# Yotsuei/ClearConverse

Measured on AMD Instinct MI355X. Metric: xRT (audio-sec/wall-sec) end-to-end, 30 s 16 kHz clips, higher is better.
Workload: dtype bf16

## Files before the change

### clearconverse_amd/csrc/sepformer.hip

```cpp
#include <math.h>
#include "../../include/ccx.h"
#include "ccx_common.h"
#include "elementwise.h"
#include <type_traits>
#include "gemm_bf16.h"
#include "model_store.h"

namespace {

typedef __attribute__((ext_vector_type(4))) short bf16x4v;

__global__ __launch_bounds__(256) void sep_encoder_kernel(const float* __restrict__ mix, long mix_stride,
                                                          const int* __restrict__ tok_utt, const int* __restrict__ tok_pos,
                                                          const int* __restrict__ utt_L, const float* __restrict__ w,
                                                          float* __restrict__ feats, int n_tok) {
  const int tok = blockIdx.x * 4 + (threadIdx.x >> 6), lane = threadIdx.x & 63;
  if (tok >= n_tok) return;
  const int u = tok_utt[tok], l = tok_pos[tok];
  float2 o = make_float2(0.f, 0.f);
  if (l < utt_L[u]) {
    const float* x = mix + (long)u * mix_stride + 8 * l;
    float xs[16];
#pragma unroll
    for (int k = 0; k < 16; k++) xs[k] = x[k];
    float a = 0.f, b = 0.f;
#pragma unroll
    for (int k = 0; k < 16; k++) {
      a = fmaf(w[(2 * lane) * 16 + k], xs[k], a);
      b = fmaf(w[(2 * lane + 1) * 16 + k], xs[k], b);
    }
    o = make_float2(fmaxf(a, 0.f), fmaxf(b, 0.f));
  }
  ((float2*)(feats + (long)tok * 128))[lane] = o;
}

__global__ void sep_block_input_kernel(const float* __restrict__ x, const float* __restrict__ hc, const int* __restrict__ tok_seq,
                                       const int* __restrict__ tok_pos, const float* __restrict__ pe, float* __restrict__ xin,
                                       float* __restrict__ h, int n_tok) {
  const long i = (long)blockIdx.x * blockDim.x + threadIdx.x;
  if (i >= (long)n_tok * 32) return;
  const int tok = (int)(i >> 5), c4 = (int)(i & 31);
  float4 v = ((const float4*)x)[i];
  if (hc) {
    const float4 a = ((const float4*)(hc + (long)tok_seq[tok] * 128))[c4];
    v.x += a.x; v.y += a.y; v.z += a.z; v.w += a.w;
  }
  ((float4*)xin)[i] = v;
  const float4 p = ((const float4*)(pe + (long)tok_pos[tok] * 128))[c4];
  ((float4*)h)[i] = make_float4(v.x + p.x, v.y + p.y, v.z + p.z, v.w + p.w);
}

__global__ __launch_bounds__(256, 2) void sep_attention_kernel(const bf16_t* __restrict__ qkv, const int* __restrict__ seq_start,
                                                            const int* __restrict__ seq_len, bf16_t* __restrict__ out,
                                                            float scale_log2e) {
  const int lane = threadIdx.x & 63, wave = threadIdx.x >> 6;
  const int seq = blockIdx.x, head = blockIdx.y * 4 + wave;
  const int s0 = seq_start[seq], len = seq_len[seq];
  const int l15 = lane & 15, h4 = lane >> 4;
  const int n_qt = (len + 15) >> 4, n_kt = n_qt;
  const bf16_t* base = qkv + (long)s0 * 384 + head * 16;

  auto load_k = [&](int kt) -> bf16x4v {
    int krow = kt * 16 + l15;
    krow = krow < len ? krow : len - 1;
    return *(const bf16x4v*)(base + 128 + (long)krow * 384 + 4 * h4);
  };
  auto load_v = [&](int kt) -> bf16x4v {
    bf16x4v v;
#pragma unroll
    for (int j = 0; j < 4; j++) {
      int vr = kt * 16 + 4 * h4 + j;
      vr = vr < len ? vr : len - 1;
      v[j] = (short)base[256 + (long)vr * 384 + l15];
    }
    return v;
  };
  const bool resident = n_kt <= 10;
  bf16x4v k_all[10], v_all[10];
  if (resident) {
#pragma unroll
    for (int t = 0; t < 10; t++) {
      const int kt = t < n_kt ? t : n_kt - 1;
      k_all[t] = load_k(kt);
      v_all[t] = load_v(kt);
    }
  }

  for (int qt = 0; qt < n_qt; qt++) {
    int qrow = qt * 16 + l15;
    qrow = qrow < len ? qrow : len - 1;
    const bf16x4v qf = *(const bf16x4v*)(base + (long)qrow * 384 + 4 * h4);
    float m_run = -1e30f, l_run = 0.f;
    f32x4 o = {0.f, 0.f, 0.f, 0.f};
    auto key_block = [&](int kt0, int nk, auto full_tag) {
      constexpr bool FULL = decltype(full_tag)::value;
      f32x4 s[10];
      bf16x4v vf[10];
#pragma unroll
      for (int t = 0; t < 10; t++) {
        if (FULL || t < nk) {
          const bf16x4v kf = resident ? k_all[t] : load_k(kt0 + t);
          s[t] = __builtin_amdgcn_mfma_f32_16x16x16bf16_1k(kf, qf, (f32x4){0.f, 0.f, 0.f, 0.f}, 0, 0, 0);
          vf[t] = resident ? v_all[t] : load_v(kt0 + t);
        }
      }
      float mx = -1e30f;
#pragma unroll
      for (int t = 0; t < 10; t++)
        if (FULL || t < nk) {
          if ((kt0 + t) * 16 + 16 > len) {
#pragma unroll
            for (int r = 0; r < 4; r++)
              if ((kt0 + t) * 16 + 4 * h4 + r >= len) s[t][r] = -INFINITY;
          }
#pragma unroll
          for (int r = 0; r < 4; r++) mx = fmaxf(mx, s[t][r]);
        }
      mx = fmaxf(mx, lane_xor16(mx));
      mx = fmaxf(mx, lane_xor32(mx));
      mx = fmaxf(m_run, mx * scale_log2e);
      const float alpha = __builtin_amdgcn_exp2f(m_run - mx);
      m_run = mx;
      float ps = 0.f;
#pragma unroll
      for (int t = 0; t < 10; t++)
        if (FULL || t < nk) {
#pragma unroll
          for (int r = 0; r < 4; r++) {
            const float pv = __builtin_amdgcn_exp2f(fmaf(s[t][r], scale_log2e, -mx));
            s[t][r] = pv;
            ps += pv;
          }
        }
      l_run = l_run * alpha + ps;
      float arow[4];
#pragma unroll
      for (int r = 0; r < 4; r++) arow[r] = __shfl(alpha, 4 * h4 + r, 64);
#pragma unroll
      for (int r = 0; r < 4; r++) o[r] *= arow[r];
#pragma unroll
      for (int t = 0; t < 10; t++)
        if (FULL || t < nk) {
          union { bf16x4v v; uint32_t u[2]; } pa;
          pa.u[0] = pack_bf16x2(s[t][0], s[t][1]);
          pa.u[1] = pack_bf16x2(s[t][2], s[t][3]);
          o = __builtin_amdgcn_mfma_f32_16x16x16bf16_1k(pa.v, vf[t], o, 0, 0, 0);
        }
    };
    for (int kt0 = 0; kt0 < n_kt; kt0 += 10) {
      const int nk = (n_kt - kt0) < 10 ? (n_kt - kt0) : 10;
      if (nk == 10) key_block(kt0, 10, std::true_type{});
      else key_block(kt0, nk, std::false_type{});
    }
    float lt = l_run + lane_xor16(l_run);
    lt += lane_xor32(lt);
#pragma unroll
    for (int r = 0; r < 4; r++) {
      const int q = qt * 16 + 4 * h4 + r;
      const float inv = 1.0f / __shfl(lt, 4 * h4 + r, 64);
      if (q < len) out[(long)(s0 + q) * 128 + head * 16 + l15] = f32_to_bf16(o[r] * inv);
    }
  }
}

__device__ __forceinline__ float2 ln_row128(const float* __restrict__ row, const float* __restrict__ g,
                                            const float* __restrict__ b, int lane) {
  const float2 v = ((const float2*)row)[lane];
  const float mean = wave_reduce_sum(v.x + v.y) * (1.0f / 128.0f);
  const float dx = v.x - mean, dy = v.y - mean;
  const float rstd = rsqrtf(wave_reduce_sum(dx * dx + dy * dy) * (1.0f / 128.0f) + 1e-6f);
  const float2 gg = ((const float2*)g)[lane], bb = ((const float2*)b)[lane];
  return make_float2(dx * rstd * gg.x + bb.x, dy * rstd * gg.y + bb.y);
}

__global__ __launch_bounds__(256) void sep_final_norm_kernel(const float* __restrict__ h, const float* __restrict__ xin,
                                                             const int* __restrict__ seq_start, const int* __restrict__ seq_len,
                                                             const float* __restrict__ ln_g, const float* __restrict__ ln_b,
                                                             const float* __restrict__ gln_g, const float* __restrict__ gln_b,
                                                             float* __restrict__ y) {
  __shared__ float red[8];
  const int seq = blockIdx.x, lane = threadIdx.x & 63, wave = threadIdx.x >> 6;
  const int s0 = seq_start[seq], len = seq_len[seq];
  float sum = 0.f;
  for (int r = wave; r < len; r += 4) {
    const float2 v = ln_row128(h + (long)(s0 + r) * 128, ln_g, ln_b, lane);
    sum += v.x + v.y;
  }
  sum = wave_reduce_sum(sum);
  if (lane == 0) red[wave] = sum;
  __syncthreads();
  const float n = (float)len * 128.0f;
  const float mean = (red[0] + red[1] + red[2] + red[3]) / n;
  float sq = 0.f;
  for (int r = wave; r < len; r += 4) {
    const float2 v = ln_row128(h + (long)(s0 + r) * 128, ln_g, ln_b, lane);
    sq += (v.x - mean) * (v.x - mean) + (v.y - mean) * (v.y - mean);
  }
  sq = wave_reduce_sum(sq);
  if (lane == 0) red[4 + wave] = sq;
  __syncthreads();
  const float rstd = 1.0f / sqrtf((red[4] + red[5] + red[6] + red[7]) / n + 1e-8f);
  const float2 gg = ((const float2*)gln_g)[lane], bb = ((const float2*)gln_b)[lane];
  for (int r = wave; r < len; r += 4) {
    const float2 v = ln_row128(h + (long)(s0 + r) * 128, ln_g, ln_b, lane);
    const float2 xi = ((const float2*)(xin + (long)(s0 + r) * 128))[lane];
    ((float2*)(y + (long)(s0 + r) * 128))[lane] =
        make_float2(gg.x * (v.x - mean) * rstd + bb.x + xi.x, gg.y * (v.y - mean) * rstd + bb.y + xi.y);
  }
}

#define FF_TOK 256
#define FF_HB 64
#define FF_P1 (FF_HB * 256)
#define FF_P2 (128 * FF_HB * 2)
#define FF_STAGE (FF_P1 + FF_P2)
#define FF_NSTAGE 4
#define FF_LDS (FF_NSTAGE * FF_STAGE + 4096)
typedef const __attribute__((address_space(1))) void* ff_gptr_t;
typedef __attribute__((address_space(3))) void* ff_lptr_t;

__device__ __forceinline__ int ff_key1(int r) { return (r & 3) | (((r >> 4) & 3) << 2); }
__device__ __forceinline__ int ff_key2(int r) { return ((r >> 1) & 1) | (((r >> 5) & 1) << 2); }

constexpr int AB_MAX_TOK = 160;
__device__ __forceinline__ int ab_off(int row, int chunk) { return row * 256 + ((chunk ^ (row & 15)) << 4); }

__global__ __launch_bounds__(512) void sep_attn_block_kernel(float* __restrict__ h, const float* __restrict__ ln_g, const float* __restrict__ ln_b,
                                                             const bf16_t* __restrict__ Wqkv, const float* __restrict__ bqkv,
                                                             const bf16_t* __restrict__ Wo, const float* __restrict__ bo,
                                                             const int* __restrict__ seq_start, const int* __restrict__ seq_len,
                                                             float scale_log2e, float eps) {
  __shared__ __attribute__((aligned(16))) char xs[AB_MAX_TOK * 256];
  const int tid = threadIdx.x, lane = tid & 63;
  const int wave = __builtin_amdgcn_readfirstlane(tid >> 6);
  const int l15 = lane & 15, h4 = lane >> 4;
  const int seq = blockIdx.x;
  const int s0 = seq_start[seq], len = seq_len[seq];
  if (len <= 0) return;
  const int n_t = (len + 15) >> 4;

  {
    const float2 g = ((const float2*)ln_g)[lane], b = ((const float2*)ln_b)[lane];
#pragma unroll
    for (int half = 0; half < 2; half++) {
      float2 v[10];
#pragma unroll
      for (int i = 0; i < 10; i++) {
        const int r = wave + 8 * (10 * half + i);
        v[i] = r < len ? ((const float2*)(h + (long)(s0 + r) * 128))[lane] : make_float2(0.f, 0.f);
      }
#pragma unroll
      for (int i = 0; i < 10; i++) {
        const int r = wave + 8 * (10 * half + i);
        const float mean = wave_reduce_sum(v[i].x + v[i].y) * (1.f / 128.f);
        const float dx = v[i].x - mean, dy = v[i].y - mean;
        const float rstd = rsqrtf(wave_reduce_sum(dx * dx + dy * dy) * (1.f / 128.f) + eps);
        uint32_t o = pack_bf16x2(dx * rstd * g.x + b.x, dy * rstd * g.y + b.y);
        if (r >= len) o = 0;
        *(uint32_t*)(xs + ab_off(r, lane >> 2) + (lane & 3) * 4) = o;
      }
    }
  }
  __syncthreads();

  bf16x4v q_all[10], k_all[10], v_all[10];
  {
    bf16x8 wq[4], wk[4];
#pragma unroll
    for (int ks = 0; ks < 4; ks++) {
      const long o = (long)(16 * wave + l15) * 128 + 32 * ks + 8 * h4;
      wq[ks] = *(const bf16x8*)(Wqkv + o);
      wk[ks] = *(const bf16x8*)(Wqkv + 128 * 128 + o);
    }
    const float4 bq = *(const float4*)(bqkv + 16 * wave + 4 * h4);
    const float4 bk = *(const float4*)(bqkv + 128 + 16 * wave + 4 * h4);
#pragma unroll
    for (int t = 0; t < 10; t++) {
      const int tt = t < n_t ? t : n_t - 1;
      f32x4 aq = {0.f, 0.f, 0.f, 0.f}, ak = aq;
#pragma unroll
      for (int ks = 0; ks < 4; ks++) {
        const bf16x8 xf = *(const bf16x8*)(xs + ab_off(16 * tt + l15, 4 * ks + h4));
        aq = __builtin_amdgcn_mfma_f32_16x16x32_bf16(wq[ks], xf, aq, 0, 0, 0);
        ak = __builtin_amdgcn_mfma_f32_16x16x32_bf16(wk[ks], xf, ak, 0, 0, 0);
      }
      union { bf16x4v v; uint32_t u[2]; } c;
      c.u[0] = pack_bf16x2(aq[0] + bq.x, aq[1] + bq.y); c.u[1] = pack_bf16x2(aq[2] + bq.z, aq[3] + bq.w);
      q_all[t] = c.v;
      c.u[0] = pack_bf16x2(ak[0] + bk.x, ak[1] + bk.y); c.u[1] = pack_bf16x2(ak[2] + bk.z, ak[3] + bk.w);
      k_all[t] = c.v;
    }
  }
  {
    bf16x8 wv[4];
#pragma unroll
    for (int ks = 0; ks < 4; ks++) wv[ks] = *(const bf16x8*)(Wqkv + 256 * 128 + (long)(16 * wave + l15) * 128 + 32 * ks + 8 * h4);
    const float bv = bqkv[256 + 16 * wave + l15];
#pragma unroll
    for (int t = 0; t < 10; t++) {
      const int tt = t < n_t ? t : n_t - 1;
      f32x4 av = {0.f, 0.f, 0.f, 0.f};
#pragma unroll
      for (int ks = 0; ks < 4; ks++) {
        const bf16x8 xf = *(const bf16x8*)(xs + ab_off(16 * tt + l15, 4 * ks + h4));
        av = __builtin_amdgcn_mfma_f32_16x16x32_bf16(xf, wv[ks], av, 0, 0, 0);
      }
      union { bf16x4v v; uint32_t u[2]; } c;
      c.u[0] = pack_bf16x2(av[0] + bv, av[1] + bv); c.u[1] = pack_bf16x2(av[2] + bv, av[3] + bv);
      v_all[t] = c.v;
    }
  }
  __syncthreads();

  for (int qt = 0; qt < n_t; qt++) {
    bf16x4v qf = q_all[0];
#pragma unroll
    for (int t = 1; t < 10; t++) qf = (t == qt) ? q_all[t] : qf;
    f32x4 sc[10];
#pragma unroll
    for (int t = 0; t < 10; t++) sc[t] = __builtin_amdgcn_mfma_f32_16x16x16bf16_1k(k_all[t], qf, (f32x4){0.f, 0.f, 0.f, 0.f}, 0, 0, 0);
    float mx = -1e30f;
#pragma unroll
    for (int t = 0; t < 10; t++) {
      if (t * 16 + 16 > len) {
#pragma unroll
        for (int r = 0; r < 4; r++)
          if (t * 16 + 4 * h4 + r >= len) sc[t][r] = -INFINITY;
      }
#pragma unroll
      for (int r = 0; r < 4; r++) mx = fmaxf(mx, sc[t][r]);
    }
    mx = fmaxf(mx, lane_xor16(mx));
    mx = fmaxf(mx, lane_xor32(mx));
    mx *= scale_log2e;
    float ps = 0.f;
    f32x4 o = {0.f, 0.f, 0.f, 0.f};
#pragma unroll
    for (int t = 0; t < 10; t++) {
#pragma unroll
      for (int r = 0; r < 4; r++) {
        const float pv = __builtin_amdgcn_exp2f(fmaf(sc[t][r], scale_log2e, -mx));
        sc[t][r] = pv;
        ps += pv;
      }
      union { bf16x4v v; uint32_t u[2]; } pa;
      pa.u[0] = pack_bf16x2(sc[t][0], sc[t][1]);
      pa.u[1] = pack_bf16x2(sc[t][2], sc[t][3]);
      o = __builtin_amdgcn_mfma_f32_16x16x16bf16_1k(pa.v, v_all[t], o, 0, 0, 0);
    }
    float lt = ps + lane_xor16(ps);
    lt += lane_xor32(lt);
#pragma unroll
    for (int r = 0; r < 4; r++) {
      const int row = qt * 16 + 4 * h4 + r;
      const float inv = 1.0f / __shfl(lt, 4 * h4 + r, 64);
      *(bf16_t*)(xs + ab_off(row, 2 * wave + (l15 >> 3)) + (l15 & 7) * 2) = f32_to_bf16(o[r] * inv);
    }
  }
  __syncthreads();

  {
    bf16x8 wo[4];
#pragma unroll
    for (int ks = 0; ks < 4; ks++) wo[ks] = *(const bf16x8*)(Wo + (long)(16 * wave + l15) * 128 + 32 * ks + 8 * h4);
    const float4 b4 = *(const float4*)(bo + 16 * wave + 4 * h4);
    for (int t = 0; t < n_t; t++) {
      const int tok = 16 * t + l15;
      float4* hp = (float4*)(h + (long)(s0 + (tok < len ? tok : len - 1)) * 128 + 16 * wave + 4 * h4);
      const float4 res = *hp;
      f32x4 acc = {0.f, 0.f, 0.f, 0.f};
#pragma unroll
      for (int ks = 0; ks < 4; ks++) {
        const bf16x8 af = *(const bf16x8*)(xs + ab_off(tok, 4 * ks + h4));
        acc = __builtin_amdgcn_mfma_f32_16x16x32_bf16(wo[ks], af, acc, 0, 0, 0);
      }
      if (tok < len) *hp = make_float4(res.x + acc[0] + b4.x, res.y + acc[1] + b4.y, res.z + acc[2] + b4.z, res.w + acc[3] + b4.w);
    }
  }
}

__global__ __launch_bounds__(512) void sep_ffn_kernel(float* __restrict__ h, const float* __restrict__ ln_g, const float* __restrict__ ln_b,
                                                      const bf16_t* __restrict__ W1, const float* __restrict__ b1,
                                                      const bf16_t* __restrict__ W2, const float* __restrict__ b2, int n_tok, int d_ffn,
                                                      float eps) {
  extern __shared__ __attribute__((aligned(16))) char ff_smem[];
  const int tid = threadIdx.x, lane = tid & 63, wave = tid >> 6;
  const int l15 = lane & 15, hq = lane >> 4;
  const int tok0 = blockIdx.x * FF_TOK + wave * 32;
  const int n_stage = d_ffn / FF_HB;
  float* b1s = (float*)(ff_smem + FF_NSTAGE * FF_STAGE);

  const bf16_t* src1[2];
  const bf16_t* src2[2];
#pragma unroll
  for (int i = 0; i < 2; i++) {
    const int r1 = (wave * 2 + i) * 4 + (lane >> 4);
    src1[i] = W1 + (long)r1 * 128 + (((lane & 15) ^ ff_key1(r1)) << 3);
    const int r2 = (wave * 2 + i) * 8 + (lane >> 3);
    src2[i] = W2 + (long)r2 * d_ffn + (((lane & 7) ^ ff_key2(r2)) << 3);
  }
  auto stage = [&](int st) {
    char* s1 = ff_smem + (st & (FF_NSTAGE - 1)) * FF_STAGE;
    char* s2 = s1 + FF_P1;
#pragma unroll
    for (int i = 0; i < 2; i++)
      __builtin_amdgcn_global_load_lds((ff_gptr_t)(src1[i] + (long)st * FF_HB * 128), (ff_lptr_t)(s1 + (wave * 2 + i) * 1024), 16, 0, 0);
#pragma unroll
    for (int i = 0; i < 2; i++)
      __builtin_amdgcn_global_load_lds((ff_gptr_t)(src2[i] + (long)st * FF_HB), (ff_lptr_t)(s2 + (wave * 2 + i) * 1024), 16, 0, 0);
  };

  bf16x8 xb[2][4];
  {
    float g[32], bt[32];
#pragma unroll
    for (int ob = 0; ob < 2; ob++)
#pragma unroll
      for (int i4 = 0; i4 < 4; i4++) {
        const float4 gv = ((const float4*)(ln_g + 64 * ob + 16 * hq))[i4], bv = ((const float4*)(ln_b + 64 * ob + 16 * hq))[i4];
        g[16 * ob + 4 * i4] = gv.x; g[16 * ob + 4 * i4 + 1] = gv.y; g[16 * ob + 4 * i4 + 2] = gv.z; g[16 * ob + 4 * i4 + 3] = gv.w;
        bt[16 * ob + 4 * i4] = bv.x; bt[16 * ob + 4 * i4 + 1] = bv.y; bt[16 * ob + 4 * i4 + 2] = bv.z; bt[16 * ob + 4 * i4 + 3] = bv.w;
      }
#pragma unroll
    for (int mt = 0; mt < 2; mt++) {
      int tok = tok0 + mt * 16 + l15;
      tok = tok < n_tok ? tok : n_tok - 1;
      const float* xr = h + (long)tok * 128 + 16 * hq;
      float v[32];
#pragma unroll
      for (int ob = 0; ob < 2; ob++)
#pragma unroll
        for (int i4 = 0; i4 < 4; i4++) {
          const float4 t = ((const float4*)(xr + 64 * ob))[i4];
          v[16 * ob + 4 * i4] = t.x; v[16 * ob + 4 * i4 + 1] = t.y; v[16 * ob + 4 * i4 + 2] = t.z; v[16 * ob + 4 * i4 + 3] = t.w;
        }
      float sm = 0.f;
#pragma unroll
      for (int c = 0; c < 32; c++) sm += v[c];
      sm += lane_xor16(sm); sm += lane_xor32(sm);
      const float mean = sm * (1.f / 128.f);
      float sq = 0.f;
#pragma unroll
      for (int c = 0; c < 32; c++) { const float d = v[c] - mean; sq = fmaf(d, d, sq); }
      sq += lane_xor16(sq); sq += lane_xor32(sq);
      const float rstd = rsqrtf(sq * (1.f / 128.f) + eps);
#pragma unroll
      for (int ks = 0; ks < 4; ks++) {
        union { bf16x8 vv; uint32_t u[4]; } cv;
#pragma unroll
        for (int e = 0; e < 4; e++) {
          const int c = 8 * ks + 2 * e;
          cv.u[e] = pack_bf16x2((v[c] - mean) * rstd * g[c] + bt[c], (v[c + 1] - mean) * rstd * g[c + 1] + bt[c + 1]);
        }
        xb[mt][ks] = cv.vv;
      }
    }
  }
  for (int i = tid; i < d_ffn; i += 512) b1s[i] = b1[i];

  f32x4 acc2[2][8];
#pragma unroll
  for (int mt = 0; mt < 2; mt++)
#pragma unroll
    for (int jo = 0; jo < 8; jo++) acc2[mt][jo] = (f32x4){0.f, 0.f, 0.f, 0.f};

  const int rq = 16 * (l15 >> 2) + (l15 & 3);
  const int k1 = l15;
  const int k2 = ((l15 >> 1) & 1) | (((l15 >> 3) & 1) << 2);
  asm volatile("s_waitcnt vmcnt(0)" ::: "memory");
  stage(0);
  if (n_stage > 1) stage(1);
  if (n_stage > 2) stage(2);
  for (int st = 0; st < n_stage; st++) {
    const int ahead = n_stage - 1 - st;
    if (ahead >= 2) asm volatile("s_waitcnt vmcnt(8)" ::: "memory");
    else if (ahead == 1) asm volatile("s_waitcnt vmcnt(4)" ::: "memory");
    else asm volatile("s_waitcnt vmcnt(0)" ::: "memory");
    asm volatile("s_waitcnt lgkmcnt(0)" ::: "memory");
    __builtin_amdgcn_s_barrier();
    if (st + 3 < n_stage) stage(st + 3);
    const char* s1 = ff_smem + (st & (FF_NSTAGE - 1)) * FF_STAGE;
    const char* s2 = s1 + FF_P1;
    f32x4 acc1[2][4];
    f32x4 bv[4];
    {
      const uint32_t baddr = (uint32_t)(uintptr_t)(ff_lptr_t)(b1s + st * FF_HB + 16 * hq);
#pragma unroll
      for (int j = 0; j < 4; j++) asm volatile("ds_read_b128 %0, %1" : "=v"(bv[j]) : "v"(baddr + 16 * j) : "memory");
    }
#pragma unroll
    for (int mt = 0; mt < 2; mt++)
#pragma unroll
      for (int j = 0; j < 4; j++) acc1[mt][j] = (f32x4){0.f, 0.f, 0.f, 0.f};
#pragma unroll
    for (int ks = 0; ks < 4; ks++) {
      const int chunk = 8 * (ks >> 1) + 2 * hq + (ks & 1);
#pragma unroll
      for (int j = 0; j < 4; j++) {
        const bf16x8 w = *(const bf16x8*)(s1 + (rq + 4 * j) * 256 + ((chunk ^ k1) << 4));
        acc1[0][j] = __builtin_amdgcn_mfma_f32_16x16x32_bf16(w, xb[0][ks], acc1[0][j], 0, 0, 0);
        acc1[1][j] = __builtin_amdgcn_mfma_f32_16x16x32_bf16(w, xb[1][ks], acc1[1][j], 0, 0, 0);
      }
    }
    asm volatile("s_waitcnt lgkmcnt(0)" ::: "memory");
    __builtin_amdgcn_sched_barrier(0);
    bf16x8 sf[2][2];
#pragma unroll
    for (int mt = 0; mt < 2; mt++)
#pragma unroll
      for (int sx = 0; sx < 2; sx++) {
        union { bf16x8 vv; uint32_t u[4]; } cv;
        const f32x4 a = acc1[mt][2 * sx] + bv[2 * sx], b = acc1[mt][2 * sx + 1] + bv[2 * sx + 1];
        cv.u[0] = pack_bf16x2(fmaxf(a[0], 0.f), fmaxf(a[1], 0.f)); cv.u[1] = pack_bf16x2(fmaxf(a[2], 0.f), fmaxf(a[3], 0.f));
        cv.u[2] = pack_bf16x2(fmaxf(b[0], 0.f), fmaxf(b[1], 0.f)); cv.u[3] = pack_bf16x2(fmaxf(b[2], 0.f), fmaxf(b[3], 0.f));
        sf[mt][sx] = cv.vv;
      }
#pragma unroll
    for (int sx = 0; sx < 2; sx++) {
      const int chunk = 2 * hq + sx;
#pragma unroll
      for (int jo = 0; jo < 8; jo++) {
        const bf16x8 w = *(const bf16x8*)(s2 + (64 * (jo >> 2) + rq + 4 * (jo & 3)) * 128 + ((chunk ^ k2) << 4));
        acc2[0][jo] = __builtin_amdgcn_mfma_f32_16x16x32_bf16(w, sf[0][sx], acc2[0][jo], 0, 0, 0);
        acc2[1][jo] = __builtin_amdgcn_mfma_f32_16x16x32_bf16(w, sf[1][sx], acc2[1][jo], 0, 0, 0);
      }
    }
  }

#pragma unroll
  for (int mt = 0; mt < 2; mt++) {
    const int tok = tok0 + mt * 16 + l15;
    if (tok >= n_tok) continue;
#pragma unroll
    for (int ob = 0; ob < 2; ob++) {
      float4* hp = (float4*)(h + (long)tok * 128 + 64 * ob + 16 * hq);
      const float4* bp = (const float4*)(b2 + 64 * ob + 16 * hq);
#pragma unroll
      for (int jp = 0; jp < 4; jp++) {
        const float4 r = hp[jp], bv = bp[jp];
        const f32x4 a = acc2[mt][4 * ob + jp];
        hp[jp] = make_float4(a[0] + bv.x + r.x, a[1] + bv.y + r.y, a[2] + bv.z + r.z, a[3] + bv.w + r.w);
      }
    }
  }
}

__global__ __launch_bounds__(128) void sep_chunk_mean_kernel(const float* __restrict__ x, float* __restrict__ mem, int seg) {
  const int chunk = blockIdx.x, c = threadIdx.x;
  const float* p = x + (long)chunk * seg * 128 + c;
  float s = 0.f;
  for (int t = 0; t < seg; t++) s += p[(long)t * 128];
  mem[(long)chunk * 128 + c] = s / (float)seg;
}

__global__ void sep_prelu_bf16_kernel(const float* __restrict__ x, const float* __restrict__ slope, bf16_t* __restrict__ out, long n4) {
  const long i = (long)blockIdx.x * blockDim.x + threadIdx.x;
  if (i >= n4) return;
  const float a = slope[0];
  const float4 v = ((const float4*)x)[i];
  uint2 o;
  o.x = pack_bf16x2(v.x >= 0 ? v.x : a * v.x, v.y >= 0 ? v.y : a * v.y);
  o.y = pack_bf16x2(v.z >= 0 ? v.z : a * v.z, v.w >= 0 ? v.w : a * v.w);
  ((uint2*)out)[i] = o;
}

__global__ __launch_bounds__(256) void sep_decoder_kernel(const float* __restrict__ feats, const float* __restrict__ fc,
                                                          const int* __restrict__ utt_tok0, const int* __restrict__ utt_L,
                                                          const int* __restrict__ utt_T, const float* __restrict__ wdec,
                                                          float* __restrict__ out, long out_stride, int n_utt) {
  const int u = blockIdx.y;
  const int l = blockIdx.x * 4 + (threadIdx.x >> 6), lane = threadIdx.x & 63;
  const int T = utt_T[u], L = utt_L[u];
  const long t0 = 8L * l;
  if (t0 >= out_stride) return;
  float2* dst = (float2*)(out + ((long)u * out_stride + t0) * 2);
  if (t0 >= T || l > L) {
    if (lane < 8 && t0 + lane < out_stride) dst[lane] = make_float2(0.f, 0.f);
    return;
  }
  float g[2][2][2];
#pragma unroll
  for (int dl = 0; dl < 2; dl++) {
    const int ll = l - dl;
    const bool ok = ll >= 0 && ll < L;
    const long tok = utt_tok0[u] + (ok ? ll : 0);
    const float2 f = ((const float2*)(feats + tok * 128))[lane];
    const float4 m = ((const float4*)(fc + tok * 256))[lane];
    const float z = ok ? 1.f : 0.f;
    g[dl][0][0] = z * f.x * fmaxf(m.x, 0.f); g[dl][0][1] = z * f.y * fmaxf(m.z, 0.f);
    g[dl][1][0] = z * f.x * fmaxf(m.y, 0.f); g[dl][1][1] = z * f.y * fmaxf(m.w, 0.f);
  }
  float4 w0[4], w1[4];
#pragma unroll
  for (int i = 0; i < 4; i++) {
    w0[i] = ((const float4*)(wdec + (2 * lane) * 16))[i];
    w1[i] = ((const float4*)(wdec + (2 * lane + 1) * 16))[i];
  }
  const float* w0f = (const float*)w0;
  const float* w1f = (const float*)w1;
  float2 res = make_float2(0.f, 0.f);
#pragma unroll
  for (int k = 0; k < 8; k++) {
    float a0 = g[0][0][0] * w0f[k] + g[0][0][1] * w1f[k];
    float a1 = g[0][1][0] * w0f[k] + g[0][1][1] * w1f[k];
    a0 += g[1][0][0] * w0f[k + 8] + g[1][0][1] * w1f[k + 8];
    a1 += g[1][1][0] * w0f[k + 8] + g[1][1][1] * w1f[k + 8];
    a0 = wave_reduce_sum(a0);
    a1 = wave_reduce_sum(a1);
    if (lane == k) res = make_float2(a0, a1);
  }
  if (lane < 8 && t0 + lane < out_stride) dst[lane] = (t0 + lane < T) ? res : make_float2(0.f, 0.f);
}

struct SepLayer {
  float *ln1_g, *ln1_b, *ln2_g, *ln2_b, *bqkv, *bo, *b1, *b2;
  bf16_t *Wqkv, *Wo, *W1, *W2;
};
struct SepBlock {
  std::vector<SepLayer> layers;
  float *lnf_g, *lnf_b, *gln_g, *gln_b;
};

}

struct ccx_sepformer {
  ccx_ctx* ctx = nullptr;
  ccx_sepformer_dims d{};
  int max_tokens = 0, max_utts = 0;
  bool finalized = false;
  ccx_dev_store store{"sepformer"};
  float *w_enc = nullptr, *w_dec = nullptr, *prelu = nullptr, *b_fc = nullptr, *pe = nullptr;
  bf16_t* W_fc = nullptr;
  std::vector<SepBlock> seg, mem;
  float *feats = nullptr, *x = nullptr, *xin = nullptr, *h = nullptr, *fc = nullptr, *memx = nullptr, *memxin = nullptr,
        *memh = nullptr, *hc = nullptr;
  bf16_t *xn = nullptr, *qkv = nullptr, *att = nullptr;
  int *tok_utt = nullptr, *tok_pos = nullptr, *tok_chunk = nullptr, *tok_cpos = nullptr, *chunk_start = nullptr,
      *chunk_len = nullptr, *utt_L = nullptr, *utt_T = nullptr, *utt_tok0 = nullptr, *utt_chunk0 = nullptr, *utt_nchunk = nullptr,
      *mem_utt = nullptr, *mem_pos = nullptr;
  int pe_len = 0;
};

namespace {

int load_block(ccx_sepformer* s, const std::string& prefix, SepBlock& B) {
  const int D = s->d.d_model, F = s->d.d_ffn;
  B.layers.resize(s->d.n_layers);
  for (int l = 0; l < s->d.n_layers; l++) {
    const std::string p = prefix + ".mdl.layers." + std::to_string(l);
    SepLayer& L = B.layers[l];
    CCX_NEED(s->store, wi, p + ".self_att.att.in_proj_weight", 3 * D, D); CCX_NEED(s->store, bi, p + ".self_att.att.in_proj_bias", 3 * D);
    CCX_NEED(s->store, wo, p + ".self_att.att.out_proj.weight", D, D); CCX_NEED(s->store, bo, p + ".self_att.att.out_proj.bias", D);
    CCX_NEED(s->store, w1, p + ".pos_ffn.ffn.0.weight", F, D); CCX_NEED(s->store, b1, p + ".pos_ffn.ffn.0.bias", F);
    CCX_NEED(s->store, w2, p + ".pos_ffn.ffn.3.weight", D, F); CCX_NEED(s->store, b2, p + ".pos_ffn.ffn.3.bias", D);
    CCX_NEED(s->store, g1, p + ".norm1.norm.weight", D); CCX_NEED(s->store, be1, p + ".norm1.norm.bias", D);
    CCX_NEED(s->store, g2, p + ".norm2.norm.weight", D); CCX_NEED(s->store, be2, p + ".norm2.norm.bias", D);
    CCX_TRY(s->store.upload_bf16(&L.Wqkv, wi->data)); CCX_TRY(s->store.upload(&L.bqkv, bi->data.data(), 3 * D));
    CCX_TRY(s->store.upload_bf16(&L.Wo, wo->data)); CCX_TRY(s->store.upload(&L.bo, bo->data.data(), D));
    CCX_TRY(s->store.upload_bf16(&L.W1, w1->data)); CCX_TRY(s->store.upload(&L.b1, b1->data.data(), F));
    CCX_TRY(s->store.upload_bf16(&L.W2, w2->data)); CCX_TRY(s->store.upload(&L.b2, b2->data.data(), D));
    CCX_TRY(s->store.upload(&L.ln1_g, g1->data.data(), D)); CCX_TRY(s->store.upload(&L.ln1_b, be1->data.data(), D));
    CCX_TRY(s->store.upload(&L.ln2_g, g2->data.data(), D)); CCX_TRY(s->store.upload(&L.ln2_b, be2->data.data(), D));
  }
  CCX_NEED(s->store, fg, prefix + ".mdl.norm.norm.weight", D); CCX_NEED(s->store, fb, prefix + ".mdl.norm.norm.bias", D);
  CCX_NEED(s->store, gg, prefix + ".norm.weight", D); CCX_NEED(s->store, gb, prefix + ".norm.bias", D);
  CCX_TRY(s->store.upload(&B.lnf_g, fg->data.data(), D)); CCX_TRY(s->store.upload(&B.lnf_b, fb->data.data(), D));
  CCX_TRY(s->store.upload(&B.gln_g, gg->data.data(), D)); CCX_TRY(s->store.upload(&B.gln_b, gb->data.data(), D));
  return CCX_OK;
}

int run_block(ccx_sepformer* s, const SepBlock& B, const float* x, const float* hc, const int* tok_seq, const int* tok_pos,
              const int* seq_start, const int* seq_len, int n_tok, int n_seq, int max_len, float* xin, float* h, float* y, hipStream_t st) {
  ccx_ctx* ctx = s->ctx;
  const int D = s->d.d_model, F = s->d.d_ffn;
  hipLaunchKernelGGL(sep_block_input_kernel, dim3(ccx_cdiv(n_tok * 32, 256)), dim3(256), 0, st, x, hc, tok_seq, tok_pos, s->pe,
                     xin, h, n_tok);
  CCX_CHECK_LAUNCH(ctx);
  const float scale_log2e = 0.25f * 1.4426950408889634f;
  const char* fenv = getenv("CCX_SEP_FUSED_ATTN");
  const bool fused = (fenv ? atoi(fenv) != 0 : true) && max_len <= AB_MAX_TOK;
  for (const SepLayer& L : B.layers) {
    GemmParams p;
    if (fused) {
      {
        ccx_prof_scope ps(ctx, st, "sep_attn_block_kernel", 2.0 * n_tok * (double)D * 4 * D + 4.0 * n_tok * (double)max_len * D,
                          2.0 * n_tok * D * 4.0 + 2.0 * 4 * D * D);
        hipLaunchKernelGGL(sep_attn_block_kernel, dim3(n_seq), dim3(512), 0, st, h, L.ln1_g, L.ln1_b, L.Wqkv, L.bqkv, L.Wo, L.bo, seq_start,
                           seq_len, scale_log2e, 1e-6f);
      }
      CCX_CHECK_LAUNCH(ctx);
    } else {
    CCX_TRY(ccx_launch_layernorm(ctx, h, D, L.ln1_g, L.ln1_b, s->xn, nullptr, D, n_tok, D, 1e-6f, st));
    memset(&p, 0, sizeof(p));
    p.A = s->xn; p.lda = D; p.W = L.Wqkv; p.ldw = D; p.M = n_tok; p.N = 3 * D; p.K = D; p.bias = L.bqkv; p.out = s->qkv; p.ldo = 3 * D;
    CCX_TRY(ccx_launch_gemm(ctx, EPI_BF16, p, st));
    {
      ccx_prof_scope ps(ctx, st, "sep_attention_kernel", 0.0, 0.0);
      hipLaunchKernelGGL(sep_attention_kernel, dim3(n_seq, s->d.n_head / 4), dim3(256), 0, st, s->qkv, seq_start, seq_len, s->att,
                         scale_log2e);
    }
    CCX_CHECK_LAUNCH(ctx);
    memset(&p, 0, sizeof(p));
    p.A = s->att; p.lda = D; p.W = L.Wo; p.ldw = D; p.M = n_tok; p.N = D; p.K = D; p.bias = L.bo; p.out = h; p.ldo = D; p.resid = h; p.ldr = D;
    CCX_TRY(ccx_launch_gemm(ctx, EPI_F32_RESID, p, st));
    }
    {
      static ccx_lds_optin optin;
      CCX_HIP(ctx, optin.ensure(ctx->device, (const void*)sep_ffn_kernel, FF_LDS));
      ccx_prof_scope ps(ctx, st, "sep_ffn_kernel", 4.0 * n_tok * (double)D * F, 2.0 * n_tok * D * 4.0 + 4.0 * D * F);
      hipLaunchKernelGGL(sep_ffn_kernel, dim3(ccx_cdiv(n_tok, FF_TOK)), dim3(512), FF_LDS, st, h, L.ln2_g, L.ln2_b, L.W1, L.b1, L.W2, L.b2,
                         n_tok, F, 1e-6f);
    }
    CCX_CHECK_LAUNCH(ctx);
  }
  hipLaunchKernelGGL(sep_final_norm_kernel, dim3(n_seq), dim3(256), 0, st, h, xin, seq_start, seq_len, B.lnf_g, B.lnf_b, B.gln_g,
                     B.gln_b, y);
  CCX_CHECK_LAUNCH(ctx);
  return CCX_OK;
}

}

extern "C" {

int ccx_sepformer_create(ccx_ctx* ctx, const ccx_sepformer_dims* dims, int max_tokens, int max_utts, ccx_sepformer** out) {
  if (!ctx) return CCX_ERR_ARG;
  CCX_REQUIRE(ctx, dims && out, "ccx_sepformer_create: null argument");
  const ccx_sepformer_dims& d = *dims;
  CCX_REQUIRE(ctx, d.n_filters == 128 && d.d_model == 128 && d.kernel == 16 && d.stride == 8 && d.n_head == 8 && d.n_spk == 2,
              "sepformer: only the resepformer-wsj02mix geometry (128 filters, k16 s8, d_model 128, 8 heads, 2 speakers) is built");
  CCX_REQUIRE(ctx, d.d_ffn % 128 == 0 && d.d_ffn <= 1024 && d.segment >= 16 && d.n_layers >= 1 && d.n_blocks >= 1, "sepformer: bad dims");
  CCX_REQUIRE(ctx, max_tokens >= d.segment && max_utts >= 1, "sepformer: capacity too small");
  ccx_sepformer* s = new ccx_sepformer();
  s->ctx = ctx; s->store.ctx = ctx; s->d = d;
  s->max_tokens = ccx_cdiv(max_tokens, d.segment) * d.segment;
  s->max_utts = max_utts;
  *out = s;
  return CCX_OK;
}

void ccx_sepformer_destroy(ccx_sepformer* s) {
  if (!s) return;
  s->store.free_all();
  delete s;
}

int ccx_sepformer_set_tensor(ccx_sepformer* s, const char* name, const float* data, int64_t numel) {
  if (!s) return CCX_ERR_ARG;
  CCX_REQUIRE(s->ctx, !s->finalized && name && data && numel > 0, "sepformer: set_tensor bad arguments");
  const std::string nm(name);
  CCX_REQUIRE(s->ctx, nm.rfind("encoder.", 0) == 0 || nm.rfind("decoder.", 0) == 0 || nm.rfind("masknet.", 0) == 0,
              "sepformer: unknown tensor name '%s'", name);
  return s->store.stage(name, data, numel);
}

int ccx_sepformer_finalize(ccx_sepformer* s) {
  if (!s) return CCX_ERR_ARG;
  CCX_REQUIRE(s->ctx, !s->finalized, "sepformer: finalize called twice");
  const ccx_sepformer_dims& d = s->d;
  const int D = d.d_model, F = d.d_ffn, N = d.n_filters;
  {
    CCX_NEED(s->store, we, "encoder.conv1d.weight", N, 1, d.kernel);
    CCX_NEED(s->store, wd, "decoder.weight", N, 1, d.kernel);
    CCX_NEED(s->store, pr, "masknet.model.output_fc.0.weight", 1);
    CCX_NEED(s->store, wf, "masknet.model.output_fc.1.weight", N * d.n_spk, D, 1);
    CCX_NEED(s->store, bf, "masknet.model.output_fc.1.bias", N * d.n_spk);
    CCX_TRY(s->store.upload(&s->w_enc, we->data));
    CCX_TRY(s->store.upload(&s->w_dec, wd->data));
    CCX_TRY(s->store.upload(&s->prelu, pr->data.data(), 1));
    CCX_TRY(s->store.upload_bf16(&s->W_fc, wf->data));
    CCX_TRY(s->store.upload(&s->b_fc, bf->data));
  }
  s->seg.resize(d.n_blocks);
  s->mem.resize(d.n_blocks > 0 ? d.n_blocks - 1 : 0);
  for (int i = 0; i < d.n_blocks; i++) {
    CCX_TRY(load_block(s, "masknet.model.seg_model." + std::to_string(i), s->seg[i]));
    if (i < d.n_blocks - 1) CCX_TRY(load_block(s, "masknet.model.mem_model." + std::to_string(i), s->mem[i]));
  }
  s->store.staged.clear();
  const int max_chunks = s->max_tokens / d.segment;
  s->pe_len = d.segment > max_chunks ? d.segment : max_chunks;
  {
    std::vector<float> pe((size_t)s->pe_len * D);
    for (int p = 0; p < s->pe_len; p++)
      for (int i = 0; i < D; i += 2) {
        const float den = expf((float)i * -(logf(10000.0f) / (float)D));
        pe[(size_t)p * D + i] = sinf((float)p * den);
        pe[(size_t)p * D + i + 1] = cosf((float)p * den);
      }
    CCX_TRY(s->store.upload(&s->pe, pe));
  }
  const size_t T = (size_t)s->max_tokens;
  CCX_TRY(s->store.alloc(&s->feats, T * D, true)); CCX_TRY(s->store.alloc(&s->x, T * D, true)); CCX_TRY(s->store.alloc(&s->xin, T * D, true)); CCX_TRY(s->store.alloc(&s->h, T * D, true));
  CCX_TRY(s->store.alloc(&s->fc, T * 2 * D, true)); CCX_TRY(s->store.alloc(&s->xn, T * D, true)); CCX_TRY(s->store.alloc(&s->qkv, T * 3 * D, true));
  CCX_TRY(s->store.alloc(&s->att, T * D, true));
  CCX_TRY(s->store.alloc(&s->memx, (size_t)max_chunks * D, true)); CCX_TRY(s->store.alloc(&s->memxin, (size_t)max_chunks * D, true));
  CCX_TRY(s->store.alloc(&s->memh, (size_t)max_chunks * D, true)); CCX_TRY(s->store.alloc(&s->hc, (size_t)max_chunks * D, true));
  CCX_TRY(s->store.alloc(&s->tok_utt, T, true)); CCX_TRY(s->store.alloc(&s->tok_pos, T, true)); CCX_TRY(s->store.alloc(&s->tok_chunk, T, true)); CCX_TRY(s->store.alloc(&s->tok_cpos, T, true));
  CCX_TRY(s->store.alloc(&s->chunk_start, (size_t)max_chunks, true)); CCX_TRY(s->store.alloc(&s->chunk_len, (size_t)max_chunks, true));
  CCX_TRY(s->store.alloc(&s->mem_utt, (size_t)max_chunks, true)); CCX_TRY(s->store.alloc(&s->mem_pos, (size_t)max_chunks, true));
  const size_t U = (size_t)s->max_utts;
  CCX_TRY(s->store.alloc(&s->utt_L, U, true)); CCX_TRY(s->store.alloc(&s->utt_T, U, true)); CCX_TRY(s->store.alloc(&s->utt_tok0, U, true)); CCX_TRY(s->store.alloc(&s->utt_chunk0, U, true));
  CCX_TRY(s->store.alloc(&s->utt_nchunk, U, true));
  s->finalized = true;
  return CCX_OK;
}

int ccx_sepformer_separate(ccx_sepformer* s, const float* mix, int64_t stride, const int* n_samples, int B, float* out,
                           void* stream_) {
  if (!s) return CCX_ERR_ARG;
  ccx_ctx* ctx = s->ctx;
  hipStream_t st = (hipStream_t)stream_;
  CCX_REQUIRE(ctx, s->finalized && mix && n_samples && out && B >= 1 && B <= s->max_utts, "sepformer_separate: bad arguments (B=%d, max %d)", B, s->max_utts);
  const ccx_sepformer_dims& d = s->d;
  const int D = d.d_model, seg = d.segment;
  std::vector<int> uL(B), uT(B), utok0(B), uchunk0(B), unchunk(B);
  int n_tok = 0, n_chunk = 0, max_nchunk = 0;
  for (int b = 0; b < B; b++) {
    CCX_REQUIRE(ctx, n_samples[b] >= d.kernel && n_samples[b] <= stride, "sepformer_separate: utterance %d has %d samples (need >= %d, <= stride)", b, n_samples[b], d.kernel);
    uT[b] = n_samples[b];
    uL[b] = (n_samples[b] - d.kernel) / d.stride + 1;
    const int rest = seg - uL[b] % seg;
    unchunk[b] = (uL[b] + rest) / seg;
    utok0[b] = n_tok; uchunk0[b] = n_chunk;
    n_tok += unchunk[b] * seg; n_chunk += unchunk[b];
    max_nchunk = unchunk[b] > max_nchunk ? unchunk[b] : max_nchunk;
  }
  CCX_REQUIRE(ctx, n_tok <= s->max_tokens, "sepformer_separate: %d tokens exceed capacity %d", n_tok, s->max_tokens);
  CCX_REQUIRE(ctx, n_chunk <= s->pe_len, "sepformer_separate: memory sequence too long");
  std::vector<int> t_utt(n_tok), t_pos(n_tok), t_chunk(n_tok), t_cpos(n_tok), c_start(n_chunk), c_len(n_chunk), m_utt(n_chunk), m_pos(n_chunk);
  for (int b = 0; b < B; b++) {
    for (int c = 0; c < unchunk[b]; c++) {
      const int cg = uchunk0[b] + c;
      c_start[cg] = utok0[b] + c * seg; c_len[cg] = seg; m_utt[cg] = b; m_pos[cg] = c;
      for (int i = 0; i < seg; i++) {
        const int t = c_start[cg] + i;
        t_utt[t] = b; t_pos[t] = c * seg + i; t_chunk[t] = cg; t_cpos[t] = i;
      }
    }
  }
#define UP(dst, vec) CCX_HIP(ctx, hipMemcpyAsync(dst, vec.data(), vec.size() * 4, hipMemcpyHostToDevice, st))
  UP(s->tok_utt, t_utt); UP(s->tok_pos, t_pos); UP(s->tok_chunk, t_chunk); UP(s->tok_cpos, t_cpos);
  UP(s->chunk_start, c_start); UP(s->chunk_len, c_len); UP(s->mem_utt, m_utt); UP(s->mem_pos, m_pos);
  UP(s->utt_L, uL); UP(s->utt_T, uT); UP(s->utt_tok0, utok0); UP(s->utt_chunk0, uchunk0); UP(s->utt_nchunk, unchunk);
#undef UP
  CCX_HIP(ctx, hipStreamSynchronize(st));

  hipLaunchKernelGGL(sep_encoder_kernel, dim3(ccx_cdiv(n_tok, 4)), dim3(256), 0, st, mix, (long)stride, s->tok_utt, s->tok_pos,
                     s->utt_L, s->w_enc, s->feats, n_tok);
  CCX_CHECK_LAUNCH(ctx);
  const float* cur = s->feats;
  const float* hc = nullptr;
  for (int i = 0; i < d.n_blocks; i++) {
    CCX_TRY(run_block(s, s->seg[i], cur, hc, s->tok_chunk, s->tok_cpos, s->chunk_start, s->chunk_len, n_tok, n_chunk, seg, s->xin, s->h,
                   s->x, st));
    cur = s->x;
    if (i < d.n_blocks - 1) {
      hipLaunchKernelGGL(sep_chunk_mean_kernel, dim3(n_chunk), dim3(128), 0, st, s->x, s->memx, seg);
      CCX_CHECK_LAUNCH(ctx);
      CCX_TRY(run_block(s, s->mem[i], s->memx, nullptr, s->mem_utt, s->mem_pos, s->utt_chunk0, s->utt_nchunk, n_chunk, B, max_nchunk, s->memxin,
                     s->memh, s->hc, st));
      hc = s->hc;
    }
  }
  hipLaunchKernelGGL(sep_prelu_bf16_kernel, dim3(ccx_cdiv(n_tok * 32, 256)), dim3(256), 0, st, s->x, s->prelu, s->xn, (long)n_tok * 32);
  CCX_CHECK_LAUNCH(ctx);
  GemmParams p;
  memset(&p, 0, sizeof(p));
  p.A = s->xn; p.lda = D; p.W = s->W_fc; p.ldw = D; p.M = n_tok; p.N = 2 * D; p.K = D; p.bias = s->b_fc; p.out = s->fc; p.ldo = 2 * D;
  CCX_TRY(ccx_launch_gemm(ctx, EPI_F32, p, st));
  hipLaunchKernelGGL(sep_decoder_kernel, dim3(ccx_cdiv(ccx_cdiv((int)stride, 8), 4), B), dim3(256), 0, st, s->feats, s->fc, s->utt_tok0, s->utt_L,
                     s->utt_T, s->w_dec, out, (long)stride, B);
  CCX_CHECK_LAUNCH(ctx);
  return CCX_OK;
}

}
```

Before: 1688.

## Prefetch all attention-block loads upfront, stage residual in LDS, fuse QKV loops

```diff
diff --git a/clearconverse_amd/csrc/sepformer.hip b/clearconverse_amd/csrc/sepformer.hip
--- a/clearconverse_amd/csrc/sepformer.hip
+++ b/clearconverse_amd/csrc/sepformer.hip
@@ -223,14 +223,45 @@
 __device__ __forceinline__ int ff_key2(int r) { return ((r >> 1) & 1) | (((r >> 5) & 1) << 2); }
 
 constexpr int AB_MAX_TOK = 160;
+constexpr int AB_XS = AB_MAX_TOK * 256;
+constexpr int AB_LDS = AB_XS + AB_MAX_TOK * 512;
 __device__ __forceinline__ int ab_off(int row, int chunk) { return row * 256 + ((chunk ^ (row & 15)) << 4); }
+__device__ __forceinline__ int ab_res_off(int row, int chunk) { return row * 512 + ((chunk ^ (row & 15)) << 4); }
+
+typedef __attribute__((ext_vector_type(2))) float f32x2v;
+__device__ __forceinline__ void ab_gload(f32x2v& d, const void* p) { asm volatile("global_load_dwordx2 %0, %1, off" : "=v"(d) : "v"(p) : "memory"); }
+__device__ __forceinline__ void ab_gload(f32x4& d, const void* p) { asm volatile("global_load_dwordx4 %0, %1, off" : "=v"(d) : "v"(p) : "memory"); }
+__device__ __forceinline__ void ab_gload(bf16x8& d, const void* p) { asm volatile("global_load_dwordx4 %0, %1, off" : "=v"(d) : "v"(p) : "memory"); }
+__device__ __forceinline__ void ab_gload(float& d, const void* p) { asm volatile("global_load_dword %0, %1, off" : "=v"(d) : "v"(p) : "memory"); }
+template <int N, typename T>
+__device__ __forceinline__ void ab_vmwait(T& d) { asm volatile("s_waitcnt vmcnt(%1)" : "+v"(d) : "n"(N) : "memory"); }
+
+#ifdef CCX_SEP_ATTN_STAMPS
+constexpr int AB_STAMP_SEQ = 2048, AB_STAMP_N = 8;
+__device__ unsigned long long ab_stamps[AB_STAMP_SEQ * AB_STAMP_N];
+#define AB_STAMP_AT(i) const unsigned long long ab_stamp_##i = __builtin_amdgcn_s_memtime();
+#define AB_STAMP_FLUSH()                                                                             \
+  do {                                                                                               \
+    asm volatile("s_waitcnt vmcnt(0)" ::: "memory");                                                 \
+    if (threadIdx.x == 0 && blockIdx.x < AB_STAMP_SEQ) {                                             \
+      unsigned long long* sp = ab_stamps + blockIdx.x * AB_STAMP_N;                                  \
+      sp[0] = ab_stamp_0; sp[1] = ab_stamp_1; sp[2] = ab_stamp_2; sp[3] = ab_stamp_3; sp[4] = ab_stamp_4; \
+      sp[5] = __builtin_amdgcn_s_memtime(); sp[6] = ab_stamp_real; sp[7] = __builtin_amdgcn_s_memrealtime(); \
+    }                                                                                                \
+  } while (0)
+#else
+#define AB_STAMP_AT(i)
+#define AB_STAMP_FLUSH() do { } while (0)
+#endif
 
 __global__ __launch_bounds__(512) void sep_attn_block_kernel(float* __restrict__ h, const float* __restrict__ ln_g, const float* __restrict__ ln_b,
                                                              const bf16_t* __restrict__ Wqkv, const float* __restrict__ bqkv,
                                                              const bf16_t* __restrict__ Wo, const float* __restrict__ bo,
                                                              const int* __restrict__ seq_start, const int* __restrict__ seq_len,
                                                              float scale_log2e, float eps) {
-  __shared__ __attribute__((aligned(16))) char xs[AB_MAX_TOK * 256];
+  extern __shared__ __attribute__((aligned(16))) char ab_smem[];
+  char* const xs = ab_smem;
+  char* const rs = ab_smem + AB_XS;
   const int tid = threadIdx.x, lane = tid & 63;
   const int wave = __builtin_amdgcn_readfirstlane(tid >> 6);
   const int l15 = lane & 15, h4 = lane >> 4;
@@ -238,79 +269,78 @@
   const int s0 = seq_start[seq], len = seq_len[seq];
   if (len <= 0) return;
   const int n_t = (len + 15) >> 4;
-
-  {
-    const float2 g = ((const float2*)ln_g)[lane], b = ((const float2*)ln_b)[lane];
-#pragma unroll
-    for (int half = 0; half < 2; half++) {
-      float2 v[10];
-#pragma unroll
-      for (int i = 0; i < 10; i++) {
-        const int r = wave + 8 * (10 * half + i);
-        v[i] = r < len ? ((const float2*)(h + (long)(s0 + r) * 128))[lane] : make_float2(0.f, 0.f);
-      }
-#pragma unroll
-      for (int i = 0; i < 10; i++) {
-        const int r = wave + 8 * (10 * half + i);
-        const float mean = wave_reduce_sum(v[i].x + v[i].y) * (1.f / 128.f);
-        const float dx = v[i].x - mean, dy = v[i].y - mean;
-        const float rstd = rsqrtf(wave_reduce_sum(dx * dx + dy * dy) * (1.f / 128.f) + eps);
-        uint32_t o = pack_bf16x2(dx * rstd * g.x + b.x, dy * rstd * g.y + b.y);
-        if (r >= len) o = 0;
-        *(uint32_t*)(xs + ab_off(r, lane >> 2) + (lane & 3) * 4) = o;
-      }
-    }
-  }
+#ifdef CCX_SEP_ATTN_STAMPS
+  const unsigned long long ab_stamp_real = __builtin_amdgcn_s_memrealtime();
+#endif
+  AB_STAMP_AT(0)
+
+  f32x2v g, b, v[20];
+  ab_gload(g, (const f32x2v*)ln_g + lane);
+  ab_gload(b, (const f32x2v*)ln_b + lane);
+#pragma unroll
+  for (int i = 0; i < 20; i++) {
+    const int r = wave + 8 * i;
+    ab_gload(v[i], (const f32x2v*)(h + (long)(s0 + (r < len ? r : len - 1)) * 128) + lane);
+  }
+  bf16x8 wq[4], wk[4], wv[4], wo[4];
+#pragma unroll
+  for (int ks = 0; ks < 4; ks++) {
+    const long o = (long)(16 * wave + l15) * 128 + 32 * ks + 8 * h4;
+    ab_gload(wq[ks], Wqkv + o);
+    ab_gload(wk[ks], Wqkv + 128 * 128 + o);
+    ab_gload(wv[ks], Wqkv + 256 * 128 + o);
+    ab_gload(wo[ks], Wo + o);
+  }
+  f32x4 bq, bk, b4;
+  float bv;
+  ab_gload(bq, bqkv + 16 * wave + 4 * h4);
+  ab_gload(bk, bqkv + 128 + 16 * wave + 4 * h4);
+  ab_gload(bv, bqkv + 256 + 16 * wave + l15);
+  ab_gload(b4, bo + 16 * wave + 4 * h4);
+
+#define AB_LN_ROW(i)                                                                                          \
+  {                                                                                                           \
+    const int r = wave + 8 * (i);                                                                             \
+    ab_vmwait<39 - (i)>(v[i]);                                                                                \
+    const float mean = wave_reduce_sum(v[i].x + v[i].y) * (1.f / 128.f);                                      \
+    const float dx = v[i].x - mean, dy = v[i].y - mean;                                                       \
+    const float rstd = rsqrtf(wave_reduce_sum(dx * dx + dy * dy) * (1.f / 128.f) + eps);                      \
+    uint32_t o = pack_bf16x2(dx * rstd * g.x + b.x, dy * rstd * g.y + b.y);                                   \
+    if (r >= len) o = 0;    \
+    *(uint32_t*)(xs + ab_off(r, lane >> 2) + (lane & 3) * 4) = o;                                             \
+    *(f32x2v*)(rs + ab_res_off(r, lane >> 1) + (lane & 1) * 8) = v[i];                                        \
+  }
+  AB_LN_ROW(0) AB_LN_ROW(1) AB_LN_ROW(2) AB_LN_ROW(3) AB_LN_ROW(4) AB_LN_ROW(5) AB_LN_ROW(6) AB_LN_ROW(7) AB_LN_ROW(8) AB_LN_ROW(9)
+  AB_LN_ROW(10) AB_LN_ROW(11) AB_LN_ROW(12) AB_LN_ROW(13) AB_LN_ROW(14) AB_LN_ROW(15) AB_LN_ROW(16) AB_LN_ROW(17) AB_LN_ROW(18) AB_LN_ROW(19)
+#undef AB_LN_ROW
+  asm volatile("s_waitcnt vmcnt(0)" : "+v"(wq[0]), "+v"(wq[1]), "+v"(wq[2]), "+v"(wq[3]), "+v"(wk[0]), "+v"(wk[1]), "+v"(wk[2]), "+v"(wk[3]) : : "memory");
+  asm volatile("" : "+v"(wv[0]), "+v"(wv[1]), "+v"(wv[2]), "+v"(wv[3]), "+v"(wo[0]), "+v"(wo[1]), "+v"(wo[2]), "+v"(wo[3]) : : "memory");
+  asm volatile("" : "+v"(bq), "+v"(bk), "+v"(bv), "+v"(b4) : : "memory");
   __syncthreads();
+  AB_STAMP_AT(1)
 
   bf16x4v q_all[10], k_all[10], v_all[10];
-  {
-    bf16x8 wq[4], wk[4];
+#pragma unroll
+  for (int t = 0; t < 10; t++) {
+    const int tt = t < n_t ? t : n_t - 1;
+    f32x4 aq = {0.f, 0.f, 0.f, 0.f}, ak = aq, av = aq;
 #pragma unroll
     for (int ks = 0; ks < 4; ks++) {
-      const long o = (long)(16 * wave + l15) * 128 + 32 * ks + 8 * h4;
-      wq[ks] = *(const bf16x8*)(Wqkv + o);
-      wk[ks] = *(const bf16x8*)(Wqkv + 128 * 128 + o);
-    }
-    const float4 bq = *(const float4*)(bqkv + 16 * wave + 4 * h4);
-    const float4 bk = *(const float4*)(bqkv + 128 + 16 * wave + 4 * h4);
-#pragma unroll
-    for (int t = 0; t < 10; t++) {
-      const int tt = t < n_t ? t : n_t - 1;
-      f32x4 aq = {0.f, 0.f, 0.f, 0.f}, ak = aq;
-#pragma unroll
-      for (int ks = 0; ks < 4; ks++) {
-        const bf16x8 xf = *(const bf16x8*)(xs + ab_off(16 * tt + l15, 4 * ks + h4));
-        aq = __builtin_amdgcn_mfma_f32_16x16x32_bf16(wq[ks], xf, aq, 0, 0, 0);
-        ak = __builtin_amdgcn_mfma_f32_16x16x32_bf16(wk[ks], xf, ak, 0, 0, 0);
-      }
-      union { bf16x4v v; uint32_t u[2]; } c;
-      c.u[0] = pack_bf16x2(aq[0] + bq.x, aq[1] + bq.y); c.u[1] = pack_bf16x2(aq[2] + bq.z, aq[3] + bq.w);
-      q_all[t] = c.v;
-      c.u[0] = pack_bf16x2(ak[0] + bk.x, ak[1] + bk.y); c.u[1] = pack_bf16x2(ak[2] + bk.z, ak[3] + bk.w);
-      k_all[t] = c.v;
-    }
-  }
-  {
-    bf16x8 wv[4];
-#pragma unroll
-    for (int ks = 0; ks < 4; ks++) wv[ks] = *(const bf16x8*)(Wqkv + 256 * 128 + (long)(16 * wave + l15) * 128 + 32 * ks + 8 * h4);
-    const float bv = bqkv[256 + 16 * wave + l15];
-#pragma unroll
-    for (int t = 0; t < 10; t++) {
-      const int tt = t < n_t ? t : n_t - 1;
-      f32x4 av = {0.f, 0.f, 0.f, 0.f};
-#pragma unroll
-      for (int ks = 0; ks < 4; ks++) {
-        const bf16x8 xf = *(const bf16x8*)(xs + ab_off(16 * tt + l15, 4 * ks + h4));
-        av = __builtin_amdgcn_mfma_f32_16x16x32_bf16(xf, wv[ks], av, 0, 0, 0);
-      }
-      union { bf16x4v v; uint32_t u[2]; } c;
-      c.u[0] = pack_bf16x2(av[0] + bv, av[1] + bv); c.u[1] = pack_bf16x2(av[2] + bv, av[3] + bv);
-      v_all[t] = c.v;
-    }
+      const bf16x8 xf = *(const bf16x8*)(xs + ab_off(16 * tt + l15, 4 * ks + h4));
+      aq = __builtin_amdgcn_mfma_f32_16x16x32_bf16(wq[ks], xf, aq, 0, 0, 0);
+      ak = __builtin_amdgcn_mfma_f32_16x16x32_bf16(wk[ks], xf, ak, 0, 0, 0);
+      av = __builtin_amdgcn_mfma_f32_16x16x32_bf16(xf, wv[ks], av, 0, 0, 0);
+    }
+    union { bf16x4v v; uint32_t u[2]; } c;
+    c.u[0] = pack_bf16x2(aq[0] + bq[0], aq[1] + bq[1]); c.u[1] = pack_bf16x2(aq[2] + bq[2], aq[3] + bq[3]);
+    q_all[t] = c.v;
+    c.u[0] = pack_bf16x2(ak[0] + bk[0], ak[1] + bk[1]); c.u[1] = pack_bf16x2(ak[2] + bk[2], ak[3] + bk[3]);
+    k_all[t] = c.v;
+    c.u[0] = pack_bf16x2(av[0] + bv, av[1] + bv); c.u[1] = pack_bf16x2(av[2] + bv, av[3] + bv);
+    v_all[t] = c.v;
   }
   __syncthreads();
+  AB_STAMP_AT(2)
 
   for (int qt = 0; qt < n_t; qt++) {
     bf16x4v qf = q_all[0];
@@ -358,25 +388,26 @@
     }
   }
   __syncthreads();
-
-  {
-    bf16x8 wo[4];
-#pragma unroll
-    for (int ks = 0; ks < 4; ks++) wo[ks] = *(const bf16x8*)(Wo + (long)(16 * wave + l15) * 128 + 32 * ks + 8 * h4);
-    const float4 b4 = *(const float4*)(bo + 16 * wave + 4 * h4);
-    for (int t = 0; t < n_t; t++) {
+  AB_STAMP_AT(3)
+
+#pragma unroll
+  for (int t = 0; t < 10; t++) {
+    if (t < n_t) {
       const int tok = 16 * t + l15;
-      float4* hp = (float4*)(h + (long)(s0 + (tok < len ? tok : len - 1)) * 128 + 16 * wave + 4 * h4);
-      const float4 res = *hp;
+      const float4 res = *(const float4*)(rs + ab_res_off(tok, 4 * wave + h4));
       f32x4 acc = {0.f, 0.f, 0.f, 0.f};
 #pragma unroll
       for (int ks = 0; ks < 4; ks++) {
         const bf16x8 af = *(const bf16x8*)(xs + ab_off(tok, 4 * ks + h4));
         acc = __builtin_amdgcn_mfma_f32_16x16x32_bf16(wo[ks], af, acc, 0, 0, 0);
       }
-      if (tok < len) *hp = make_float4(res.x + acc[0] + b4.x, res.y + acc[1] + b4.y, res.z + acc[2] + b4.z, res.w + acc[3] + b4.w);
-    }
-  }
+      if (tok < len)
+        *(float4*)(h + (long)(s0 + tok) * 128 + 16 * wave + 4 * h4) =
+            make_float4(res.x + acc[0] + b4[0], res.y + acc[1] + b4[1], res.z + acc[2] + b4[2], res.w + acc[3] + b4[3]);
+    }
+  }
+  AB_STAMP_AT(4)
+  AB_STAMP_FLUSH();
 }
 
 __global__ __launch_bounds__(512) void sep_ffn_kernel(float* __restrict__ h, const float* __restrict__ ln_g, const float* __restrict__ ln_b,
@@ -669,6 +700,27 @@
   return CCX_OK;
 }
 
+#ifdef CCX_SEP_ATTN_STAMPS
+int ab_dump_stamps(ccx_ctx* ctx, int n_seq, hipStream_t st) {
+  static int seen = 0;
+  const char* path = getenv("CCX_SEP_ATTN_STAMPS_OUT");
+  if (!path || n_seq < 1000 || n_seq > AB_STAMP_SEQ || ++seen != 121) return CCX_OK;
+  std::vector<unsigned long long> hs((size_t)n_seq * AB_STAMP_N);
+  CCX_HIP(ctx, hipStreamSynchronize(st));
+  CCX_HIP(ctx, hipMemcpyFromSymbol(hs.data(), HIP_SYMBOL(ab_stamps), hs.size() * 8));
+  FILE* f = fopen(path, "w");
+  if (!f) return CCX_OK;
+  fprintf(f, "# block  memtime: entry ln_done qkv_done attn_done stores_issued stores_retired   memrealtime: entry end\n");
+  for (int i = 0; i < n_seq; i++) {
+    fprintf(f, "%d", i);
+    for (int j = 0; j < AB_STAMP_N; j++) fprintf(f, " %llu", hs[(size_t)i * AB_STAMP_N + j]);
+    fprintf(f, "\n");
+  }
+  fclose(f);
+  return CCX_OK;
+}
+#endif
+
 int run_block(ccx_sepformer* s, const SepBlock& B, const float* x, const float* hc, const int* tok_seq, const int* tok_pos,
               const int* seq_start, const int* seq_len, int n_tok, int n_seq, int max_len, float* xin, float* h, float* y, hipStream_t st) {
   ccx_ctx* ctx = s->ctx;
@@ -685,10 +737,15 @@
       {
         ccx_prof_scope ps(ctx, st, "sep_attn_block_kernel", 2.0 * n_tok * (double)D * 4 * D + 4.0 * n_tok * (double)max_len * D,
                           2.0 * n_tok * D * 4.0 + 2.0 * 4 * D * D);
-        hipLaunchKernelGGL(sep_attn_block_kernel, dim3(n_seq), dim3(512), 0, st, h, L.ln1_g, L.ln1_b, L.Wqkv, L.bqkv, L.Wo, L.bo, seq_start,
-                           seq_len, scale_log2e, 1e-6f);
+        static ccx_lds_optin optin;
+        CCX_HIP(ctx, optin.ensure(ctx->device, (const void*)sep_attn_block_kernel, AB_LDS));
+        hipLaunchKernelGGL(sep_attn_block_kernel, dim3(n_seq), dim3(512), AB_LDS, st, h, L.ln1_g, L.ln1_b, L.Wqkv, L.bqkv, L.Wo, L.bo,
+                           seq_start, seq_len, scale_log2e, 1e-6f);
       }
       CCX_CHECK_LAUNCH(ctx);
+#ifdef CCX_SEP_ATTN_STAMPS
+      CCX_TRY(ab_dump_stamps(ctx, n_seq, st));
+#endif
     } else {
     CCX_TRY(ccx_launch_layernorm(ctx, h, D, L.ln1_g, L.ln1_b, s->xn, nullptr, D, n_tok, D, 1e-6f, st));
     memset(&p, 0, sizeof(p));
```

New measurement: 1654. 0.98x the previous value.
